# TomasDelaney/A-Deep-Reinforcement-Learning-Enabled-Soft-Exoskeleton-for-Parkinson-s-Patients

Measured on AMD Instinct MI355X. Metric: env steps/sec (batched exo sim) + TD7 grad-steps/sec at 1/2/4/8 MI355X, higher is better.
Workload: dtype f64 sim + bf16 TD7

## Files before the change

a-deep-reinforcement-learning-enabled-soft-exoskeleton-for-parkinson-s-patients_amd/csrc/exo_env.hip:

```cpp
#include <hip/hip_runtime.h>

#include <cmath>
#include <cstdio>
#include <cstring>
#include <string>
#include <vector>

#include "exo_amd.h"
#include "exo_model.h"

using namespace exo;

namespace {

__device__ __forceinline__ double cfg(const Dev &S, int k, int e) { return S.cfg[(size_t)k * S.N + e]; }

__device__ __forceinline__ double wave_min(double v) {
#pragma unroll
    for (int o = 32; o > 0; o >>= 1) v = fmin(v, __shfl_xor(v, o, 64));
    return v;
}
__device__ __forceinline__ double wave_max(double v) {
#pragma unroll
    for (int o = 32; o > 0; o >>= 1) v = fmax(v, __shfl_xor(v, o, 64));
    return v;
}

struct Draws {
    const double *buf;
    uint64_t seed;
    uint32_t env, episode;
    __device__ __forceinline__ double operator()(int p) const {
        return buf ? buf[p] : philox_u01(seed, env, episode, (uint32_t)p);
    }
};

template <int n>
__device__ __forceinline__ void invert(double *a , double *inv) {
#pragma unroll
    for (int i = 0; i < n * n; ++i) inv[i] = (i % (n + 1) == 0) ? 1.0 : 0.0;
#pragma unroll
    for (int k = 0; k < n; ++k) {
        int p = k;
        double best = fabs(a[k * n + k]);
#pragma unroll
        for (int i = k + 1; i < n; ++i) {
            const double v = fabs(a[i * n + k]);
            if (v > best) { best = v; p = i; }
        }
#pragma unroll
        for (int i = k + 1; i < n; ++i) {
            const bool sw = p == i;
#pragma unroll
            for (int j = 0; j < n; ++j) {
                const double t = a[k * n + j], u = inv[k * n + j];
                a[k * n + j] = sw ? a[i * n + j] : t;
                a[i * n + j] = sw ? t : a[i * n + j];
                inv[k * n + j] = sw ? inv[i * n + j] : u;
                inv[i * n + j] = sw ? u : inv[i * n + j];
            }
        }
        const double r = 1.0 / a[k * n + k];
#pragma unroll
        for (int j = 0; j < n; ++j) { a[k * n + j] *= r; inv[k * n + j] *= r; }
#pragma unroll
        for (int i = 0; i < n; ++i) {
            if (i == k) continue;
            const double m = a[i * n + k];
#pragma unroll
            for (int j = 0; j < n; ++j) { a[i * n + j] -= m * a[k * n + j]; inv[i * n + j] -= m * inv[k * n + j]; }
        }
    }
}

template <int EPW, int TS>
__device__ void reset_group(const Dev &S, const Urdf &U, int e, const double *draws, uint64_t seed, float *obs) {
#pragma clang fp contract(off)
    constexpr int NT = EPW * TS, NW = NT / 64;
    static_assert(NT % 64 == 0 && 64 % EPW == 0, "whole wavefronts, a slot's threads spread over lanes");
    const int el = threadIdx.x % EPW, tl = threadIdx.x / EPW, w = threadIdx.x / 64;
    const bool on = e >= 0;
    const int ee = on ? e : 0;
    if (on && tl == 0 && S.pend) S.pend[e] = 0;
    const int N = S.N, L = on ? S.L[ee] : 0, seq = S.seq[ee];
    const uint32_t ep = S.episode[ee];
    const Draws D{draws, seed, (uint32_t)ee, ep};
// ... 97 lines not shown
        const double sr = cfg(S, C_SHIFT, ee);
        for (int j = tl; j < 42; j += TS) {
            const double v = -sr + (sr - (-sr)) * D(pI + 147 + j);
            sShift[el][j] = v;
            S.shift[(size_t)j * N + e] = v;
        }
    }
    __syncthreads();
    if (on) {
        for (int k = tl; k < NSYM; k += TS) {
            int r = 0, c = 0;
#pragma unroll
            for (int q = 0; q < NSYM; ++q)
                if (q == k) { r = SYM_R[q]; c = SYM_C[q]; }
            S.dnz[(size_t)k * N + e] = sD[el][r * 7 + c];
            S.snz[(size_t)k * N + e] = sS[el][r * 7 + c];
        }
        if (tl == 0) {
            double a3[9], i3[9], a4[16], i4[16];
            for (int i = 0; i < 3; ++i)
                for (int j = 0; j < 3; ++j) a3[i * 3 + j] = sI[el][B1[i] * 7 + B1[j]];
            for (int i = 0; i < 4; ++i)
                for (int j = 0; j < 4; ++j) a4[i * 4 + j] = sI[el][B2[i] * 7 + B2[j]];
            invert<3>(a3, i3);
            invert<4>(a4, i4);
            for (int i = 0; i < 3; ++i)
                for (int j = i; j < 3; ++j) sInv[el][B1U[i][j]] = i3[i * 3 + j];
            for (int i = 0; i < 4; ++i)
                for (int j = i; j < 4; ++j) sInv[el][B2U[i][j]] = i4[i * 4 + j];
        }
    }
    __syncthreads();
    if (!on) return;
    for (int k = tl; k < NINV; k += TS) S.iinv[(size_t)k * N + e] = sInv[el][k];
    if (tl != 0) return;
    const double ar = cfg(S, C_ACTR, e), lo = 1 - ar, hi = 1 + ar;
    const double maxS = cfg(S, C_MAXS0, e) * (lo + (hi - lo) * D(pI + 189));
    const double maxE = cfg(S, C_MAXE0, e) * (lo + (hi - lo) * D(pI + 190));
    S.maxSE[e] = maxS;
    S.maxSE[(size_t)N + e] = maxE;
    S.counts[e] = 2;
    S.episode[e] = ep + 1;

    double q[5], act[14][3], ref[6], refc[6];
#pragma unroll
    for (int j = 0; j < 5; ++j) q[j] = S.phys_q[(size_t)j * N + e];
#pragma unroll
    for (int j = 0; j < 6; ++j) refc[j] = S.ref[(size_t)j * N + e];
    link_coms(U, q, act, ref);
    float *o = obs ? obs + (size_t)e * OBS : nullptr;
    float ob[OBS];
#pragma unroll
    for (int i = 0; i < 14; ++i) ob[i] = 0.0f;
    const double tn[4] = {10, 10, 10, 5};
#pragma unroll
    for (int t = 0; t < 3; ++t)
#pragma unroll
        for (int i = 0; i < 4; ++i) ob[14 + t * 4 + i] = (float)(sTrem[el][t][i] / tn[i]);
#pragma unroll
    for (int j = 0; j < 7; ++j)
#pragma unroll
        for (int a = 0; a < 3; ++a) {
            const double p = act[2 * j + 1][a] + sShift[el][(2 * j + 1) * 3 + a];
            const double rc = (j < 2) ? refc[3 + a] : refc[a];
            const double rn = (j < 2) ? ref[3 + a] : ref[a];
            ob[26 + j * 3 + a] = (float)(p - rc);
            const float pv = (float)(p - rn);
            ob[47 + j * 3 + a] = pv;
            S.posv[(size_t)(j * 3 + a) * N + e] = pv;
        }
#pragma unroll
    for (int j = 0; j < 6; ++j) {
        ob[68 + j] = (float)ref[j];
        ob[74 + j] = (float)ref[j];
        S.ref[(size_t)j * N + e] = ref[j];
    }
    if (o) {
#pragma unroll
        for (int i = 0; i < OBS; i += 4) *reinterpret_cast<float4 *>(o + i) = make_float4(ob[i], ob[i + 1], ob[i + 2], ob[i + 3]);
    }
}

constexpr int RESET_EPW = 16, RESET_TS = 32;
__global__ __launch_bounds__(RESET_EPW *RESET_TS) void exo_reset_kernel(Dev S, Urdf U, const uint8_t *mask,
                                                                        const int32_t *ids, int n,
                                                                        const double *draws, int draw_stride,
                                                                        uint64_t seed, float *obs) {
    const int slot = blockIdx.x * RESET_EPW + (int)threadIdx.x % RESET_EPW;
    int e = -1;
    if (ids) {
        if (slot < n) e = ids[slot];
    } else if (slot < S.N && !(mask && !mask[slot])) {
        e = slot;
    }
    reset_group<RESET_EPW, RESET_TS>(S, U, e, draws && slot < n ? draws + (size_t)slot * draw_stride : nullptr,
                                     seed, obs);
}

__global__ __launch_bounds__(64) void exo_reset_list_kernel(Dev S, Urdf U, const int32_t *ids,
                                                            const int32_t *n_ids, uint64_t seed, float *obs) {
    const int n = *n_ids;
    for (int k = blockIdx.x; k < n; k += gridDim.x) reset_group<1, 64>(S, U, ids[k], nullptr, seed, obs);
}

__global__ __launch_bounds__(256) void exo_step_kernel(Dev S, Urdf U, const float *__restrict__ act,
                                                       float *__restrict__ obs, float *__restrict__ rew,
                                                       uint8_t *__restrict__ done, float *__restrict__ info,
                                                       const uint8_t *__restrict__ active) {
    const int gid = blockIdx.x * blockDim.x + threadIdx.x;
    const int e = gid >> 1, role = gid & 1;
    if (e >= S.N) return;
    const int N = S.N, c = S.counts[e], L = S.L[e];
    if ((active && !active[e]) || c >= L - 1) return;

    double T[7];
    {
        const double maxS = S.maxSE[e], maxE = S.maxSE[(size_t)N + e];
        double F[7];
        const float *a = act + (size_t)e * ACT;
#pragma unroll
        for (int j = 0; j < 7; ++j) F[j] = (((double)a[j] + 1) / 2) * (j < 2 ? maxE : maxS);
        double q[5], ak[14][3], refn[6], refo[6];
#pragma unroll
        for (int j = 0; j < 5; ++j) q[j] = S.phys_q[(size_t)j * N + e];
#pragma unroll
        for (int j = 0; j < 6; ++j) refo[j] = S.ref[(size_t)j * N + e];
        if (S.mb_q) {
            double qp[14];
#pragma unroll
            for (int j = 0; j < 14; ++j) qp[j] = S.mb_q[(size_t)(5 + j) * N + e];
            link_coms(U, q, ak, refn, qp);
        } else {
            link_coms(U, q, ak, refn);
        }
#pragma unroll
        for (int k = 0; k < 14; ++k)
#pragma unroll
            for (int a3 = 0; a3 < 3; ++a3) ak[k][a3] += S.shift[(size_t)(k * 3 + a3) * N + e];

        double tau[7][3];
#pragma unroll
        for (int j = 0; j < 7; ++j) {
            const double *k1 = ak[2 * j], *k2 = ak[2 * j + 1];
            const double dx = (k2[0] + 5) - (k1[0] + 5), dy = (k2[1] + 5) - (k1[1] + 5), dz = (k2[2] + 5) - (k1[2] + 5);
            const double fx = cos_atan2(dy, dx) * F[j], fy = cos_atan2(dx, dy) * F[j], fz = cos_atan2(dz, dx) * F[j];
            const double *rn = (j < 2) ? &refn[3] : &refn[0];
            const double r0 = rn[0] - k2[0], r1 = rn[1] - k2[1], r2 = rn[2] - k2[2];
            tau[j][0] = fy * r2 - fz * r1;
            tau[j][1] = fz * r0 - fx * r2;
            tau[j][2] = fx * r1 - fy * r0;
        }
        double at[4];
        at[0] = tau[2][1] + tau[3][1] + tau[4][1] + tau[6][1] + tau[5][1];
        at[1] = tau[2][0] + tau[3][0] + tau[4][0] + tau[6][0] + tau[5][0];
        at[2] = tau[2][2] + tau[3][2] + tau[4][2] + tau[6][2] + tau[5][2];
        at[3] = fabs(tau[0][1]) - fabs(tau[1][1]);

        double tr[7], Ta[7];
#pragma unroll
        for (int j = 0; j < 7; ++j) {
            tr[j] = S.tremor[((size_t)c * 7 + j) * N + e];
            Ta[j] = tr[j] + (j < 4 ? at[j] : 0.0);
            T[j] = role == 0 ? Ta[j] : tr[j];
        }

        if (role == 0) {
// ... 239 lines not shown
__global__ void eval_metrics_kernel(Dev S, const float *__restrict__ info, const uint8_t *__restrict__ stepped,
                                    double L1, double L2, float *__restrict__ counters) {
    const int e = blockIdx.x * blockDim.x + threadIdx.x;
    if (e >= S.N || (stepped && !stepped[e])) return;
    const float *in = info + (size_t)e * INFO;
    const int seq = S.seq[e];
    bool all_sup = true, any_sup = false;
    for (int j = 0; j < 7; ++j) {
        if (!((seq >> j) & 1)) continue;
        const double ref = in[21 + j];
        double tr = (fabs((double)in[7 + j]) - fabs(ref)) / fabs(ref + 1e-10) * 100.0;
        if (!isfinite(tr)) tr = 0.0;
        all_sup &= tr <= 0.0;
        any_sup |= tr <= 0.0;
    }
    const int cnt = S.counts[e];
    const double *imu = S.imu + (size_t)S.motion[e] * 5 * S.Lmax;
    const int col[5] = {2, 3, 4, 0, 1};
    double q0[7], q1[7], q2[7];
    for (int j = 0; j < 7; ++j) {
        const int js = j == 0 ? 1 : (j == 1 ? 0 : j);
        const double o = j < 5 ? imu[col[j] * S.Lmax + cnt] * (PI / 180) : 0.0;
        q0[j] = o;
        q1[j] = (double)in[14 + js] * (PI / 180) + o;
        q2[j] = (double)in[28 + js] * (PI / 180) + o;
    }
    double p0[3], p1[3], p2[3];
    dh_end_effector(q0, L1, L2, p0);
    dh_end_effector(q1, L1, L2, p1);
    dh_end_effector(q2, L1, L2, p2);
    const double ds = sqrt((p1[0] - p0[0]) * (p1[0] - p0[0]) + (p1[1] - p0[1]) * (p1[1] - p0[1]) +
                           (p1[2] - p0[2]) * (p1[2] - p0[2]));
    const double du = sqrt((p2[0] - p0[0]) * (p2[0] - p0[0]) + (p2[1] - p0[1]) * (p2[1] - p0[1]) +
                           (p2[2] - p0[2]) * (p2[2] - p0[2]));
    const double total = (ds - du) / du * 100.0;
    float *cn = counters + (size_t)e * 5;
    if (all_sup) cn[0] += 1;
    if (any_sup) cn[1] += 1;
    if (total < 0) {
        cn[2] += 1;
        cn[4] += (float)total;
    } else {
        cn[3] += 1;
    }
}

__global__ __launch_bounds__(1024) void active_advance_kernel(const uint8_t *__restrict__ table, int rows, int n,
                                                              long long *k, uint8_t *__restrict__ active,
                                                              int32_t *count, const float *__restrict__ rew,
                                                              double *__restrict__ score) {
    __shared__ int wsum[16];
    const long long k0 = *k;
    const long long kk = k0 + 1 < rows ? k0 + 1 : rows - 1;
    int c = 0;
    for (int e = threadIdx.x; e < n; e += blockDim.x) {
        const uint8_t v = table[(size_t)kk * n + e];
        if (score) score[e] += active[e] ? (double)rew[e] : 0.0;
        active[e] = v;
        c += v != 0;
    }
    for (int o = 32; o > 0; o >>= 1) c += __shfl_xor(c, o, 64);
    if ((threadIdx.x & 63) == 0) wsum[threadIdx.x >> 6] = c;
    __syncthreads();
    if (threadIdx.x == 0) {
        *k = kk;
        if (count) {
            int t = 0;
            for (int w = 0; w < (int)(blockDim.x >> 6); ++w) t += wsum[w];
            *count = t;
        }
    }
}

struct exo_ctx {
    int device = 0;
    int N = 0, n_motions = 0, Lmax = 0;
    uint64_t seed = 0;
    Dev S{};
    Urdf U{};
    std::vector<int32_t> L_host, motion_host;
    std::vector<double> imu_host;
    std::vector<void *> allocs;
    float *obs_scratch = nullptr;
    int step_variant = EXO_STEP_AUTO;
    int physics = EXO_PHYS_IDEAL;
    MbModel mb{};
    double *mb_q = nullptr, *mb_qd = nullptr, *mb_tgt = nullptr;
    uint8_t *mb_flag = nullptr;
    unsigned long long *step_clock = nullptr;
    std::string err;
};

namespace {

struct DeviceGuard {
    int prev = -1;
    explicit DeviceGuard(int dev) {
        if (hipGetDevice(&prev) == hipSuccess && prev != dev) (void)hipSetDevice(dev);
        else prev = -1;
    }
    ~DeviceGuard() {
        if (prev >= 0) (void)hipSetDevice(prev);
    }
};

int fail(exo_ctx *c, int code, const std::string &msg) {
    if (c) c->err = msg;
    return code;
}

int check(exo_ctx *c, hipError_t e, const char *what) {
    if (e == hipSuccess) return EXO_OK;
    return fail(c, EXO_EDEVICE, std::string(what) + ": " + hipGetErrorString(e));
}

template <class T>
T *dalloc(exo_ctx *c, size_t n) {
    void *p = nullptr;
    if (hipMalloc(&p, n * sizeof(T)) != hipSuccess) return nullptr;
    (void)hipMemset(p, 0, n * sizeof(T));
    c->allocs.push_back(p);
    return static_cast<T *>(p);
}

}

namespace {
template <class T>
int read1(exo_ctx *c, const T *base, size_t idx, T *out) {
    return check(c, hipMemcpy(out, base + idx, sizeof(T), hipMemcpyDeviceToHost), "read-back");
}
template <class T>
int write1(exo_ctx *c, T *base, size_t idx, T v) {
    return check(c, hipMemcpy(base + idx, &v, sizeof(T), hipMemcpyHostToDevice), "write");
}
}

extern "C" {

int exo_create(const exo_env_config *cfgs, int32_t n_envs, const double *motion_angles, const int32_t *motion_lengths,
               int32_t n_motions, int32_t max_len, uint64_t seed, int32_t device, exo_ctx **out) {
    if (!out || !cfgs || !motion_angles || !motion_lengths || n_envs <= 0 || n_motions <= 0 || max_len <= 2 ||
        max_len > MAX_L)
        return EXO_EINVAL;
    *out = nullptr;
    for (int m = 0; m < n_motions; ++m)
        if (motion_lengths[m] < 4 || motion_lengths[m] > max_len) return EXO_EINVAL;
    std::vector<double> cfg((size_t)C_COUNT * n_envs);
    std::vector<int32_t> seq(n_envs), L(n_envs), mot(n_envs);
    for (int e = 0; e < n_envs; ++e) {
        const exo_env_config &c = cfgs[e];
        if (c.motion < 0 || c.motion >= n_motions) return EXO_EINVAL;
        int bits = 0, n = 0;
        for (int i = 0; i < 7; ++i) {
            if (c.tremor_sequence[i] != 0 && c.tremor_sequence[i] != 1) return EXO_EINVAL;
            bits |= c.tremor_sequence[i] << i;
            n += c.tremor_sequence[i];
        }
        if (n == 0) return EXO_EINVAL;
        seq[e] = bits;
        mot[e] = c.motion;
        L[e] = motion_lengths[c.motion];
        const double v[C_COUNT] = {c.tremor_amplitude_range[0], c.tremor_amplitude_range[1],
                                   c.first_harmonics_interval[0], c.first_harmonics_interval[1],
                                   c.second_harmonics_interval[0], c.second_harmonics_interval[1],
                                   c.max_force_shoulder, c.max_force_elbow, c.dr_actuator_end_pos_shift,
                                   c.dr_actuator_range, c.matrix_noise_fraction,
                                   n * 0.5 + 0.9 + 0.05 + 0.05 + 0.5, (double)n};
        for (int k = 0; k < C_COUNT; ++k) cfg[(size_t)k * n_envs + e] = v[k];
    }
    exo_ctx *c = new exo_ctx();
    c->device = device;
    c->N = n_envs;
    c->n_motions = n_motions;
    c->Lmax = max_len;
    c->seed = seed;
    c->L_host = L;
    c->motion_host = mot;
    c->imu_host.assign(motion_angles, motion_angles + (size_t)n_motions * 5 * max_len);
    build_urdf(c->U);
    DeviceGuard g(device);
    const size_t N = n_envs;
    Dev &S = c->S;
    S.N = n_envs; S.n_motions = n_motions; S.Lmax = max_len;
    int32_t *motion_d = dalloc<int32_t>(c, N), *L_d = dalloc<int32_t>(c, N), *seq_d = dalloc<int32_t>(c, N);
    double *cfg_d = dalloc<double>(c, cfg.size()), *imu_d = dalloc<double>(c, c->imu_host.size());
    S.tremor = dalloc<double>(c, (size_t)max_len * 7 * N);
    S.iinv = dalloc<double>(c, NINV * N);
    S.dnz = dalloc<double>(c, NSYM * N);
    S.snz = dalloc<double>(c, NSYM * N);
    S.shift = dalloc<double>(c, 42 * N);
    S.maxSE = dalloc<double>(c, 2 * N);
    S.episode = dalloc<uint32_t>(c, N);
    S.counts = dalloc<int32_t>(c, N);
    S.phys_q = dalloc<double>(c, 5 * N);
    S.ref = dalloc<double>(c, 6 * N);
    S.posv = dalloc<float>(c, 21 * N);
    S.prev_a = dalloc<double>(c, 7 * N);
    S.prev2_a = dalloc<double>(c, 7 * N);
    S.err = dalloc<int32_t>(c, 1);
    S.viol = dalloc<int32_t>(c, N);
    c->obs_scratch = dalloc<float>(c, N * OBS);
    for (void *p : c->allocs)
        if (!p) { exo_destroy(c); return EXO_ENOMEM; }
    if (!motion_d || !L_d || !seq_d || !cfg_d || !imu_d || !S.tremor || !S.iinv ||
        !S.dnz || !S.snz || !S.shift || !S.maxSE || !S.episode || !S.counts || !S.phys_q || !S.ref || !S.posv ||
        !S.prev_a || !S.prev2_a || !S.err || !S.viol || !c->obs_scratch) {
        exo_destroy(c);
        return EXO_ENOMEM;
    }
    S.motion = motion_d; S.L = L_d; S.seq = seq_d; S.cfg = cfg_d; S.imu = imu_d;
    exo_set_tremor_model(c, nullptr, EXO_TREMOR_SIGN_PER_SAMPLE);
    hipError_t e = hipMemcpy(motion_d, mot.data(), N * 4, hipMemcpyHostToDevice);
    if (e == hipSuccess) e = hipMemcpy(L_d, L.data(), N * 4, hipMemcpyHostToDevice);
    if (e == hipSuccess) e = hipMemcpy(seq_d, seq.data(), N * 4, hipMemcpyHostToDevice);
    if (e == hipSuccess) e = hipMemcpy(cfg_d, cfg.data(), cfg.size() * 8, hipMemcpyHostToDevice);
    if (e == hipSuccess) e = hipMemcpy(imu_d, c->imu_host.data(), c->imu_host.size() * 8, hipMemcpyHostToDevice);
    if (e != hipSuccess) { exo_destroy(c); return EXO_EDEVICE; }
    int rc = exo_reset(c, nullptr, c->obs_scratch, nullptr);
    if (rc == EXO_OK) rc = check(c, hipDeviceSynchronize(), "exo_create");
    if (rc != EXO_OK) { exo_destroy(c); return rc; }
    *out = c;
    return EXO_OK;
}

int exo_reset(exo_ctx *c, const uint8_t *mask_dev, float *obs_dev, void *stream) {
    if (!c) return EXO_EINVAL;
    DeviceGuard g(c->device);
    hipLaunchKernelGGL(exo_reset_kernel, dim3((c->N + RESET_EPW - 1) / RESET_EPW), dim3(RESET_EPW * RESET_TS), 0,
                       (hipStream_t)stream, c->S, c->U, mask_dev, (const int32_t *)nullptr, 0,
                       (const double *)nullptr, 0, c->seed, obs_dev);
    return check(c, hipGetLastError(), "exo_reset");
}

int exo_reset_from_draws(exo_ctx *c, const int32_t *env_ids_host, int32_t n, const double *draws_host, float *obs_dev,
                         void *stream) {
    if (!c || !env_ids_host || !draws_host || n <= 0) return EXO_EINVAL;
    for (int k = 0; k < n; ++k)
        if (env_ids_host[k] < 0 || env_ids_host[k] >= c->N) return fail(c, EXO_EINVAL, "env id out of range");
    DeviceGuard g(c->device);
    const int stride = EXO_DRAWS_PER_EPISODE(c->Lmax);
    int32_t *ids = nullptr;
    double *dr = nullptr;
    if (hipMalloc(&ids, n * 4) != hipSuccess || hipMalloc(&dr, (size_t)n * stride * 8) != hipSuccess) {
        (void)hipFree(ids);
        return fail(c, EXO_ENOMEM, "exo_reset_from_draws: out of memory");
    }
    hipStream_t s = (hipStream_t)stream;
    hipError_t e = hipMemcpyAsync(ids, env_ids_host, n * 4, hipMemcpyHostToDevice, s);
    if (e == hipSuccess) e = hipMemcpyAsync(dr, draws_host, (size_t)n * stride * 8, hipMemcpyHostToDevice, s);
    if (e == hipSuccess) {
        hipLaunchKernelGGL(exo_reset_kernel, dim3((n + RESET_EPW - 1) / RESET_EPW), dim3(RESET_EPW * RESET_TS), 0,
                           s, c->S, c->U, (const uint8_t *)nullptr, ids, n, dr, stride, c->seed, obs_dev);
        e = hipGetLastError();
    }
    if (e == hipSuccess) e = hipStreamSynchronize(s);
    (void)hipFree(ids);
    (void)hipFree(dr);
    return check(c, e, "exo_reset_from_draws");
}

namespace {
__global__ void step_clock_kernel(unsigned long long *clk, int end) {
    const unsigned long long t = wall_clock64();
    if (!end) {
        clk[0] = t;
    } else {
        clk[1] += t - clk[0];
        clk[2] += 1;
    }
}
}

int exo_step(exo_ctx *c, const float *act_dev, float *obs_dev, float *rew_dev, uint8_t *done_dev, float *info_dev,
             const uint8_t *active_dev, void *stream) {
    return exo_step_carry(c, act_dev, obs_dev, rew_dev, done_dev, info_dev, active_dev, nullptr, stream);
}

namespace {
bool rows_variant(const exo_ctx *c) {
    return c->step_variant == EXO_STEP_ROWS_SHARED || c->step_variant == EXO_STEP_ROWS ||
           (c->step_variant == EXO_STEP_AUTO && c->N <= 16384);
}

__global__ __launch_bounds__(1024) void budget_advance_kernel(const int32_t *counts, const int32_t *L,
                                                              const uint8_t *pend, int n, uint8_t *active,
                                                              int32_t *count, int32_t *remaining,
                                                              long long *steps_total) {
    __shared__ int wsum[2][16];
    int a = 0, rem = 0;
    for (int e = threadIdx.x; e < n; e += blockDim.x) {
        const bool run = counts[e] < L[e] - 1, p = pend[e] != 0;
        active[e] = run && !p;
        a += run && !p;
        rem += run || p;
    }
    for (int o = 32; o > 0; o >>= 1) {
        a += __shfl_xor(a, o, 64);
        rem += __shfl_xor(rem, o, 64);
    }
    if ((threadIdx.x & 63) == 0) {
        wsum[0][threadIdx.x >> 6] = a;
        wsum[1][threadIdx.x >> 6] = rem;
    }
    __syncthreads();
    if (threadIdx.x == 0) {
        int ta = 0, tr = 0;
        for (int w = 0; w < (int)(blockDim.x >> 6); ++w) {
            ta += wsum[0][w];
            tr += wsum[1][w];
        }
        if (steps_total) *steps_total += *count;
        *count = ta;
        *remaining = tr;
    }
}

__global__ __launch_bounds__(1024) void episode_advance_kernel(const int32_t *counts, const int32_t *L,
                                                               const uint8_t *pend, int n, uint8_t *active,
                                                               int32_t *count, int32_t *reset_ids,
                                                               long long *steps_total) {
    __shared__ int wsum[16];
    __shared__ int nres;
    if (threadIdx.x == 0) nres = 0;
    __syncthreads();
    int a = 0;
    for (int e = threadIdx.x; e < n; e += blockDim.x) {
        const bool fin = counts[e] >= L[e] - 1, p = pend && pend[e] != 0;
        if (fin && !p) reset_ids[atomicAdd(&nres, 1)] = e;
        const bool run = !p;
        active[e] = run;
        a += run;
    }
    for (int o = 32; o > 0; o >>= 1) a += __shfl_xor(a, o, 64);
    if ((threadIdx.x & 63) == 0) wsum[threadIdx.x >> 6] = a;
    __syncthreads();
    if (threadIdx.x == 0) {
        int ta = 0;
        for (int w = 0; w < (int)(blockDim.x >> 6); ++w) ta += wsum[w];
        if (steps_total) *steps_total += *count;
        *count = ta;
        reset_ids[n] = nres;
    }
}
}

int exo_set_step_budget(exo_ctx *c, int32_t budget) {
    if (!c || budget < 0) return EXO_EINVAL;
    DeviceGuard g(c->device);
    if (budget > 0 && (!rows_variant(c) || c->physics != EXO_PHYS_IDEAL))
        return fail(c, EXO_EINVAL, "exo_set_step_budget: row-parallel step kernels and idealised physics only");
    int rc = check(c, hipDeviceSynchronize(), "exo_set_step_budget");
    if (rc) return rc;
    if (budget == 0) {
        if (c->S.pend) {
            std::vector<uint8_t> p(c->N);
            rc = check(c, hipMemcpy(p.data(), c->S.pend, c->N, hipMemcpyDeviceToHost), "exo_set_step_budget");
            if (rc) return rc;
            for (uint8_t v : p)
                if (v) return fail(c, EXO_EINVAL, "exo_set_step_budget: a solve is still pending");
        }
        c->S.budget = 0;
        return EXO_OK;
    }
    if (!c->S.pend) {
        c->S.pend = dalloc<uint8_t>(c, c->N);
        c->S.rk = dalloc<double>(c, (size_t)RK_FIELDS * c->N);
        if (!c->S.pend || !c->S.rk) return fail(c, EXO_ENOMEM, "exo_set_step_budget: out of memory");
    }
    c->S.budget = budget;
    return EXO_OK;
}

int exo_budget_advance(exo_ctx *c, uint8_t *active_dev, int32_t *count_dev, int32_t *remaining_dev,
                       int64_t *steps_total_dev, void *stream) {
    if (!c || !active_dev || !count_dev || !remaining_dev) return EXO_EINVAL;
    if (!c->S.pend) return fail(c, EXO_EINVAL, "exo_budget_advance: no step budget set");
    DeviceGuard g(c->device);
    hipLaunchKernelGGL(budget_advance_kernel, dim3(1), dim3(1024), 0, (hipStream_t)stream, c->S.counts, c->S.L,
                       c->S.pend, c->N, active_dev, count_dev, remaining_dev, (long long *)steps_total_dev);
    return check(c, hipGetLastError(), "exo_budget_advance");
}

int exo_episode_advance(exo_ctx *c, uint8_t *active_dev, int32_t *count_dev, int32_t *reset_ws_dev,
                        int64_t *steps_total_dev, float *obs_dev, void *stream) {
    if (!c || !active_dev || !count_dev || !reset_ws_dev || !obs_dev) return EXO_EINVAL;
    DeviceGuard g(c->device);
    const hipStream_t s = (hipStream_t)stream;
    hipLaunchKernelGGL(episode_advance_kernel, dim3(1), dim3(1024), 0, s, c->S.counts, c->S.L, c->S.pend, c->N,
                       active_dev, count_dev, reset_ws_dev, (long long *)steps_total_dev);
    hipError_t e = hipGetLastError();
    if (e == hipSuccess) {
        hipLaunchKernelGGL(exo_reset_list_kernel, dim3(std::min(c->N, 64)), dim3(64), 0, s, c->S, c->U, reset_ws_dev,
                           reset_ws_dev + c->N, c->seed, obs_dev);
        e = hipGetLastError();
    }
    return check(c, e, "exo_episode_advance");
}

int exo_step_carry(exo_ctx *c, const float *act_dev, float *obs_dev, float *rew_dev, uint8_t *done_dev,
                   float *info_dev, const uint8_t *active_dev, const float *obs_cur_dev, void *stream) {
    if (!c || !act_dev || !obs_dev || !rew_dev || !done_dev) return EXO_EINVAL;
    DeviceGuard g(c->device);
    const bool shared = c->step_variant == EXO_STEP_ROWS_SHARED;
    const bool rows = rows_variant(c);
    if (c->S.budget > 0 && (!rows || c->physics != EXO_PHYS_IDEAL))
        return fail(c, EXO_EINVAL, "exo_step: the step budget needs the row-parallel kernel and idealised physics");
    hipError_t e = hipSuccess;
    if (c->step_clock) {
        hipLaunchKernelGGL(step_clock_kernel, dim3(1), dim3(1), 0, (hipStream_t)stream, c->step_clock, 0);
        e = hipGetLastError();
    }
    if (e != hipSuccess) {
    } else if (rows) {
        e = launch_exo_step_rp(c->S, c->U, act_dev, obs_dev, rew_dev, done_dev, info_dev, active_dev,
                               (hipStream_t)stream, shared, obs_cur_dev);
    } else {
        const int threads = 256, lanes = 2 * c->N;
        hipLaunchKernelGGL(exo_step_kernel, dim3((lanes + threads - 1) / threads), dim3(threads), 0,
                           (hipStream_t)stream, c->S, c->U, act_dev, obs_dev, rew_dev, done_dev, info_dev, active_dev);
        e = hipGetLastError();
    }
    if (e == hipSuccess && c->physics == EXO_PHYS_MULTIBODY)
        e = launch_exo_multibody(c->S, c->U, c->mb, c->S.mb_tgt, c->S.mb_flag, 1, (hipStream_t)stream);
    if (e == hipSuccess && c->step_clock) {
        hipLaunchKernelGGL(step_clock_kernel, dim3(1), dim3(1), 0, (hipStream_t)stream, c->step_clock, 1);
        e = hipGetLastError();
    }
    return check(c, e, "exo_step");
}

void exo_multibody_default_params(exo_mb_params *p) {
    if (!p) return;
    p->gravity = 9.81;
    p->kp = 0.1;
    p->kd = 1.0;
    p->motor_impulse = 1e5 * DT;
    p->passive_impulse = 1.0;
    p->limit_impulse = 100.0;
    p->erp = 0.2;
    p->lin_damp = 0.04;
    p->ang_damp = 0.04;
    p->max_vel = 100.0;
    p->iters = 50;
}

int exo_set_physics(exo_ctx *c, int32_t mode, const exo_mb_params *params) {
    if (!c || (mode != EXO_PHYS_IDEAL && mode != EXO_PHYS_MULTIBODY)) return EXO_EINVAL;
    if (mode == EXO_PHYS_MULTIBODY && c->S.budget > 0)
        return fail(c, EXO_EINVAL, "exo_set_physics: the step budget needs idealised physics");
    exo_mb_params p;
    exo_multibody_default_params(&p);
    if (params) p = *params;
    if (p.iters < 0 || p.iters > 100000 || !(p.motor_impulse >= 0) || !(p.passive_impulse >= 0) ||
        !(p.limit_impulse >= 0) || !(p.max_vel > 0))
        return fail(c, EXO_EINVAL, "exo_set_physics: invalid multibody parameters");
    DeviceGuard g(c->device);
    const size_t N = c->N;
    int rc = check(c, hipDeviceSynchronize(), "exo_set_physics");
    if (rc) return rc;
    if (mode == EXO_PHYS_IDEAL) {
        c->physics = mode;
        c->S.mb_q = c->S.mb_qd = c->S.mb_tgt = nullptr;
        c->S.mb_flag = nullptr;
        return EXO_OK;
    }
    if (!c->mb_q) {
        c->mb_q = dalloc<double>(c, NJ * N);
        c->mb_qd = dalloc<double>(c, NJ * N);
        c->mb_tgt = dalloc<double>(c, 5 * N);
        c->mb_flag = dalloc<uint8_t>(c, N);
// ... 265 lines not shown
```

a-deep-reinforcement-learning-enabled-soft-exoskeleton-for-parkinson-s-patients_amd/csrc/lap.hip:

```cpp
#include <hip/hip_runtime.h>

#include <algorithm>
#include <cstdint>
#include <cstdlib>
#include <string>

#include "lap_chain.h"
#include "philox.h"
#include "exo_amd.h"

namespace {

constexpr int UPD_THREADS = 1024;

__device__ __forceinline__ float *stratum_tree(float *tree, int s, int cap) { return tree + (size_t)s * 2 * cap; }

constexpr int TOPN = 8192;
template <int NTOP = TOPN>
__device__ bool propagate_top(float *T, int cap, int levels, const int32_t *slot, int n, float *top) {
    int lv = 1;
    for (; lv <= levels && ((2 * cap) >> lv) > NTOP / 2; ++lv) {
        __syncthreads();
        for (int k = threadIdx.x; k < n; k += blockDim.x) {
            const int node = (cap + slot[k]) >> lv;
            T[node] = T[2 * node] + T[2 * node + 1];
        }
    }
    __syncthreads();
    if (lv > levels) return false;
    const int lim = min(NTOP, 2 * cap);
    if (blockDim.x == UPD_THREADS) {
        constexpr int PER = NTOP / UPD_THREADS;
        float v[PER];
#pragma unroll
        for (int j = 0; j < PER; ++j) {
            const int i = threadIdx.x + j * UPD_THREADS;
            v[j] = i < lim ? T[i] : 0.0f;
        }
#pragma unroll
        for (int j = 0; j < PER; ++j) {
            const int i = threadIdx.x + j * UPD_THREADS;
            if (i < lim) top[i] = v[j];
        }
    } else {
        for (int i = threadIdx.x; i < lim; i += blockDim.x) top[i] = T[i];
    }
    for (; lv <= levels; ++lv) {
        __syncthreads();
        for (int k = threadIdx.x; k < n; k += blockDim.x) {
            const int node = (cap + slot[k]) >> lv;
            top[node] = top[2 * node] + top[2 * node + 1];
        }
    }
    __syncthreads();
    const int wb = min(NTOP / 2, cap);
    for (int i = 1 + threadIdx.x; i < wb; i += blockDim.x) T[i] = top[i];
    __syncthreads();
    return true;
}
__device__ void propagate(float *T, int cap, int levels, const int32_t *slot, int n) {
    __shared__ float top[TOPN];
    propagate_top(T, cap, levels, slot, n, top);
}

__device__ void propagate_span(float *T, int cap, int levels, int capacity, int first, int count) {
    __shared__ float top[TOPN];
    if (count <= 0) return;
    int a0 = first, e0 = first + count, a1 = 0, e1 = 0;
    if (count >= capacity) {
        a0 = 0;
        e0 = capacity;
    } else if (e0 > capacity) {
        e1 = e0 - capacity;
        e0 = capacity;
    }
    int lv = 1;
    for (; lv <= levels && ((2 * cap) >> lv) > TOPN / 2; ++lv) {
        __syncthreads();
        const int lo0 = (cap + a0) >> lv, n0 = ((cap + e0 - 1) >> lv) - lo0 + 1;
        const int lo1 = (cap + a1) >> lv, n1 = e1 > a1 ? ((cap + e1 - 1) >> lv) - lo1 + 1 : 0;
        for (int k = threadIdx.x; k < n0 + n1; k += blockDim.x) {
            const int node = k < n0 ? lo0 + k : lo1 + k - n0;
            T[node] = T[2 * node] + T[2 * node + 1];
        }
    }
    __syncthreads();
    if (lv > levels) return;
    const int lim = min(TOPN, 2 * cap);
    for (int i = threadIdx.x; i < lim; i += blockDim.x) top[i] = T[i];
    for (; lv <= levels; ++lv) {
        __syncthreads();
        const int lo0 = (cap + a0) >> lv, n0 = ((cap + e0 - 1) >> lv) - lo0 + 1;
        const int lo1 = (cap + a1) >> lv, n1 = e1 > a1 ? ((cap + e1 - 1) >> lv) - lo1 + 1 : 0;
        for (int k = threadIdx.x; k < n0 + n1; k += blockDim.x) {
            const int node = k < n0 ? lo0 + k : lo1 + k - n0;
            top[node] = top[2 * node] + top[2 * node + 1];
        }
    }
    __syncthreads();
    const int wb = min(TOPN / 2, cap);
    for (int i = 1 + threadIdx.x; i < wb; i += blockDim.x) T[i] = top[i];
    __syncthreads();
}

constexpr int SPAN_LDS = 4096;
constexpr int SPAN_LEVELS = 32;
__device__ bool propagate_span_lds(float *T, int cap, int levels, int capacity, int first, int count,
                                   float *buf , float *edge ) {
    const int a = cap + first, e = cap + first + count - 1;
    if (count <= 0 || first + count > capacity || count > SPAN_LDS - 2 || levels >= SPAN_LEVELS) return false;
    const int t = threadIdx.x;
    if (t < 2 * levels) {
        const int lv = t >> 1, right = t & 1;
        const int lo = a >> lv, hi = e >> lv;
        if (!right && (lo & 1)) edge[t] = T[lo - 1];
        if (right && !(hi & 1)) edge[t] = T[hi + 1];
    }
    float *A = buf, *B = buf + SPAN_LDS;
    {
        const int base = a & ~1;
        for (int c = a + t; c <= e; c += blockDim.x) A[c - base] = T[c];
    }
    __syncthreads();
    if (t == 0) {
        if (a & 1) A[0] = edge[0];
        if (!(e & 1)) A[(e | 1) - (a & ~1)] = edge[1];
    }
    for (int lv = 1; lv <= levels; ++lv) {
        __syncthreads();
        const int lo = a >> lv, hi = e >> lv, cbase = (a >> (lv - 1)) & ~1, nbase = lo & ~1;
        for (int node = lo + t; node <= hi; node += blockDim.x) {
            const int c = 2 * node - cbase;
            const float v = A[c] + A[c + 1];
            T[node] = v;
            B[node - nbase] = v;
        }
        if (t == 0 && lv < levels) {
            if (lo & 1) B[0] = edge[2 * lv];
            if (!(hi & 1)) B[(hi | 1) - nbase] = edge[2 * lv + 1];
        }
        float *tmp = A;
        A = B;
        B = tmp;
    }
    __syncthreads();
    return true;
}

constexpr int ADD_CHUNK = 4096;
__global__ __launch_bounds__(UPD_THREADS) void lap_add_kernel(float *tree, const float *maxp, int cap, int levels,
                                                              int capacity, const int32_t *stratum,
                                                              const int32_t *slot, int n) {
    const int s = blockIdx.x;
    float *T = stratum_tree(tree, s, cap);
    __shared__ int32_t mine[ADD_CHUNK];
    __shared__ int count;
    const float p = *maxp;
    for (int base = 0; base < n; base += ADD_CHUNK) {
        if (threadIdx.x == 0) count = 0;
        __syncthreads();
        const int end = min(n, base + ADD_CHUNK);
        for (int k = base + threadIdx.x; k < end; k += blockDim.x) {
            if (stratum[k] != s) continue;
            const int sl = slot[k];
            if (sl < 0 || sl >= capacity) continue;
            T[cap + sl] = p;
            mine[atomicAdd(&count, 1)] = sl;
        }
        __syncthreads();
        propagate(T, cap, levels, mine, count);
    }
}

constexpr int MAXLV = 24;
template <class At>
__device__ __forceinline__ float prefix_sum(At at, int cap, int levels, int sz) {
    if (sz >= cap) return at(1);
    float v[MAXLV];
#pragma unroll
    for (int j = 0; j < MAXLV; ++j) {
        v[j] = 0.0f;
        if (j < levels) {
            const int lv = levels - 1 - j;
            const float x = at(2 * ((1 << j) | (sz >> (lv + 1))));
            v[j] = ((sz >> lv) & 1) ? x : 0.0f;
// ... 597 lines not shown
            const int r = rk[jj];
            if (jj + 1 == m) {
                carry_r = r;
                carry_i = ri[jj];
                carry_J = soff + jj;
                sl[jj] = -1;
                continue;
            }
            const long long mr = mult_below(count0 + r, E);
            const bool win = (long long)rk[jj + 1] > mr * E - count0;
            const int slot = win ? slot_of(r) : -1;
            sl[jj] = slot;
            if (win && part == 0) T[cap + slot] = p;
        }
        __syncthreads();
        if (cpart >= 0) {
            const int j0 = ((cpart - soff) % KC + KC) % KC;
            copy_rows<VEC>(st, state, action, next_state, reward, done, action_scale, ri, sl, s, capacity, j0, KC, m,
                           t, UPD_THREADS);
        }
        offset += chunk_tot;
        soff += m;
        __syncthreads();
    }
    if (t == 0) {
        carry_slot = -1;
        if (carry_r >= 0) {
            carry_slot = slot_of(carry_r);
            if (part == 0) T[cap + carry_slot] = p;
        }
    }
    __syncthreads();
    if (carry_slot >= 0 && wv == 0 && carry_J % KC == cpart)
        copy_rows<VEC>(st, state, action, next_state, reward, done, action_scale, &carry_i, &carry_slot, s, capacity,
                       0, 1, 1, lane, 64);
    const int n_act = offset;
    if (part == 0 && n_act > 0) {
        __shared__ float span_buf[2 * SPAN_LDS], span_edge[2 * SPAN_LEVELS];
        __syncthreads();
        const long long last = mult_below(count0 + n_act - 1, E) - m0;
        const int cnt = (int)min(last + 1, (long long)capacity);
        if (!propagate_span_lds(T, cap, levels, capacity, (int)ptr0, cnt, span_buf, span_edge))
            propagate_span(T, cap, levels, capacity, (int)ptr0, cnt);
    }
    __syncthreads();
    __shared__ int last;
    if (t == 0) {
        last = atomicAdd(ticket, 1u) == (uint32_t)(E * K - 1);
        if (last) {
            const long long na = mult_below(count0 + n_act, E) - m0;
            const long long size = min(size0 + na, (long long)capacity);
            for (int q = 0; q < E; ++q) ring_size[q] = (int32_t)size;
            ref[0] = (ptr0 + na) % capacity;
            ref[1] = count0 + n_act;
            ref[2] = size;
            *ticket = 0u;
        }
    }
    __syncthreads();
    if (!last || !adv.table) return;
    const long long k0 = *adv.k;
    const long long kk = k0 + 1 < adv.rows ? k0 + 1 : adv.rows - 1;
    int c = 0;
    for (int e = t; e < n; e += UPD_THREADS) {
        const uint8_t v = adv.table[(size_t)kk * n + e];
        if (adv.score) adv.score[e] += adv.active[e] ? (double)reward[e] : 0.0;
        adv.active[e] = v;
        c += v != 0;
    }
    for (int o = 32; o > 0; o >>= 1) c += __shfl_xor(c, o, 64);
    __shared__ int wc[UPD_THREADS / 64];
    if (lane == 0) wc[wv] = c;
    __syncthreads();
    if (t == 0) {
        *adv.k = kk;
        if (adv.count) {
            int tot = 0;
            for (int w = 0; w < UPD_THREADS / 64; ++w) tot += wc[w];
            *adv.count = tot;
        }
    }
}

__global__ __launch_bounds__(256) void lap_store_copy_kernel(lap_storage_desc st, const float *state,
                                                             const float *action, const float *next_state,
                                                             const float *reward, const uint8_t *done,
                                                             float action_scale, int n, const int32_t *row_of) {
    const int i = blockIdx.x * 4 + (threadIdx.x >> 6), lane = threadIdx.x & 63;
    if (i >= n) return;
    const long r = row_of[i];
    if (r < 0) return;
    const int sd = st.state_dim, ad = st.action_dim;
    for (int k = lane; k < sd; k += 64) {
        st.state[r * sd + k] = state[(long)i * sd + k];
        st.next_state[r * sd + k] = next_state[(long)i * sd + k];
    }
    for (int k = lane; k < ad; k += 64) st.action[r * ad + k] = action[(long)i * ad + k] / action_scale;
    if (lane == 0) {
        st.reward[r] = reward[i];
        st.not_done[r] = 1.0f - (done[i] ? 1.0f : 0.0f);
    }
}

__device__ __forceinline__ void sample_descend(const float *tree, int cap, int levels, int capacity, float ud,
                                               const int32_t *size, int batch, int d, int lane, int32_t *idx,
                                               const lap_storage_desc &st, float *o_state, float *o_action,
                                               float *o_next, float *o_reward, float *o_not_done) {
    const int s = d / batch;
    const float *T = tree + (size_t)s * 2 * cap;
    const int sz = size[s];
    const float val = ud * prefix_total(T, cap, levels, sz);
    const int node = descend_from([T](int n) { return T[n]; }, val, 1, 0, levels);
    int i = node - cap;
    if (i >= sz) i = sz > 0 ? sz - 1 : 0;
    if (lane == 0) idx[d] = i;
    const long r = (long)s * (capacity + 1) + i;
    const int sd = st.state_dim, ad = st.action_dim;
    for (int k = lane; k < sd; k += 64) {
        o_state[(long)d * sd + k] = st.state[r * sd + k];
        o_next[(long)d * sd + k] = st.next_state[r * sd + k];
    }
    for (int k = lane; k < ad; k += 64) o_action[(long)d * ad + k] = st.action[r * ad + k];
    if (lane == 0) {
        o_reward[d] = st.reward[r];
        o_not_done[d] = st.not_done[r];
    }
}

struct SampleRng {
    uint64_t seed;
    uint32_t tag;
    unsigned long long *counter;
    uint32_t *ticket;
};

__global__ __launch_bounds__(256) void lap_sample_gather_kernel(const float *tree, int cap, int levels, int capacity,
                                                                const float *u, const int32_t *size, int batch,
                                                                int total, int32_t *idx, lap_storage_desc st,
                                                                float *o_state, float *o_action, float *o_next,
                                                                float *o_reward, float *o_not_done, SampleRng rng) {
    const int d = blockIdx.x * 4 + (threadIdx.x >> 6), lane = threadIdx.x & 63;
    if (rng.counter) {
        const unsigned long long call = *rng.counter;
        __syncthreads();
        if (threadIdx.x == 0) {
            __threadfence();
            if (atomicAdd(rng.ticket, 1u) == gridDim.x - 1) {
                *rng.counter = call + 1ull;
                *rng.ticket = 0u;
            }
        }
        if (d >= total) return;
        uint32_t r[4];
        philox_block(rng.seed, rng.tag, call, (uint32_t)d, r);
        sample_descend(tree, cap, levels, capacity, u01_open_hi(r[0]), size, batch, d, lane, idx, st, o_state,
                       o_action, o_next, o_reward, o_not_done);
        return;
    }
    if (d >= total) return;
    sample_descend(tree, cap, levels, capacity, u[d], size, batch, d, lane, idx, st, o_state, o_action, o_next,
                   o_reward, o_not_done);
}


#ifndef LAP_TOPN_US
#define LAP_TOPN_US 8192
// ... 589 lines not shown

extern "C" {

int32_t lap_tree_floats(int32_t n_strata, int32_t capacity) {
    int cap = 1;
    while (cap < capacity) cap <<= 1;
    return n_strata * 2 * cap;
}

int lap_init(const lap_tree_desc *t, void *stream) {
    if (!valid(t)) return EXO_EINVAL;
    hipError_t e = hipMemsetAsync(t->tree, 0, (size_t)t->n_strata * 2 * t->cap * sizeof(float), (hipStream_t)stream);
    if (e != hipSuccess) return EXO_EDEVICE;
    hipLaunchKernelGGL(lap_init_kernel, dim3(1), dim3(1), 0, (hipStream_t)stream, t->max_priority);
    return rc(hipGetLastError());
}

int lap_add(const lap_tree_desc *t, const int32_t *stratum, const int32_t *slot, int32_t n, void *stream) {
    if (!valid(t) || !stratum || !slot || n < 0) return EXO_EINVAL;
    if (n == 0) return EXO_OK;
    hipLaunchKernelGGL(lap_add_kernel, dim3(t->n_strata), dim3(UPD_THREADS), 0, (hipStream_t)stream, t->tree,
                       t->max_priority, t->cap, levels_of(t), t->capacity, stratum, slot, n);
    return rc(hipGetLastError());
}

int lap_sample(const lap_tree_desc *t, const float *u, const int32_t *size, int32_t batch, int32_t *idx, void *stream) {
    if (!valid(t) || !u || !size || !idx || batch <= 0) return EXO_EINVAL;
    const int th = 128;
    hipLaunchKernelGGL(lap_sample_kernel, dim3((batch + th - 1) / th, t->n_strata), dim3(th), 0, (hipStream_t)stream,
                       t->tree, t->cap, levels_of(t), u, size, batch, idx);
    return rc(hipGetLastError());
}

int lap_update(const lap_tree_desc *t, const int32_t *idx, const float *prio, int32_t batch, void *stream) {
    if (!valid(t) || !idx || !prio || batch <= 0) return EXO_EINVAL;
    hipLaunchKernelGGL(lap_update_kernel, dim3(t->n_strata), dim3(UPD_THREADS), 0, (hipStream_t)stream, t->tree,
                       t->max_priority, t->cap, levels_of(t), idx, prio, batch);
    return rc(hipGetLastError());
}

int lap_reset_max(const lap_tree_desc *t, void *stream) {
    if (!valid(t)) return EXO_EINVAL;
    hipError_t e = hipMemsetAsync(t->max_priority, 0, sizeof(float), (hipStream_t)stream);
    if (e != hipSuccess) return EXO_EDEVICE;
    hipLaunchKernelGGL(lap_reset_max_kernel, dim3(256), dim3(1024), 0, (hipStream_t)stream, t->tree, t->max_priority,
                       t->cap, t->n_strata);
    return rc(hipGetLastError());
}

int lap_totals(const lap_tree_desc *t, float *out, void *stream) {
    if (!valid(t) || !out) return EXO_EINVAL;
    hipLaunchKernelGGL(lap_totals_kernel, dim3((t->n_strata + 63) / 64), dim3(64), 0, (hipStream_t)stream, t->tree,
                       t->cap, t->n_strata, out);
    return rc(hipGetLastError());
}

int lap_store_batch(const lap_tree_desc *t, const lap_storage_desc *st, const float *state, const float *action,
                    const float *next_state, const float *reward, const uint8_t *done, const int32_t *strata,
                    const uint8_t *active, float action_scale, int32_t n, int32_t *row_ws, void *stream) {
    if (!valid(t) || !st || !st->state || !st->action || !st->next_state || !st->reward || !st->not_done ||
        !st->ptr || !st->size || st->state_dim <= 0 || st->action_dim <= 0 || !state || !action || !next_state ||
        !reward || !done || !strata || !row_ws || n < 0 || action_scale == 0.0f)
        return EXO_EINVAL;
    if (n == 0) return EXO_OK;
    const char *fused_var = getenv("EXO_LAP_STORE_FUSED");
    const bool fused_env = fused_var && fused_var[0] == '1';
    if (fused_env && n <= STORE_FUSED_MAX && n <= t->capacity) {
        const bool vec = (st->state_dim & 3) == 0 &&
                         ((reinterpret_cast<uintptr_t>(state) | reinterpret_cast<uintptr_t>(next_state) |
                           reinterpret_cast<uintptr_t>(st->state) | reinterpret_cast<uintptr_t>(st->next_state)) &
                          15) == 0;
        if (vec)
            hipLaunchKernelGGL(lap_store_fused_kernel<true>, dim3(t->n_strata), dim3(UPD_THREADS), 0,
                               (hipStream_t)stream, t->tree, t->max_priority, t->cap, levels_of(t), t->capacity,
                               st->ptr, st->size, strata, active, n, row_ws, *st, state, action, next_state, reward,
                               done, action_scale);
        else
            hipLaunchKernelGGL(lap_store_fused_kernel<false>, dim3(t->n_strata), dim3(UPD_THREADS), 0,
                               (hipStream_t)stream, t->tree, t->max_priority, t->cap, levels_of(t), t->capacity,
                               st->ptr, st->size, strata, active, n, row_ws, *st, state, action, next_state, reward,
                               done, action_scale);
        return rc(hipGetLastError());
    }
    if (n > 4 * STORE_CHUNK)
        hipLaunchKernelGGL(lap_store_rank_kernel<16>, dim3(t->n_strata), dim3(UPD_THREADS), 0, (hipStream_t)stream,
                           t->tree, t->max_priority, t->cap, levels_of(t), t->capacity, st->ptr, st->size, strata,
                           active, n, row_ws);
    else
        hipLaunchKernelGGL(lap_store_rank_kernel<4>, dim3(t->n_strata), dim3(UPD_THREADS), 0, (hipStream_t)stream,
                           t->tree, t->max_priority, t->cap, levels_of(t), t->capacity, st->ptr, st->size, strata,
                           active, n, row_ws);
    if (hipGetLastError() != hipSuccess) return EXO_EDEVICE;
    hipLaunchKernelGGL(lap_store_copy_kernel, dim3((n + 3) / 4), dim3(256), 0, (hipStream_t)stream, *st, state,
                       action, next_state, reward, done, action_scale, n, row_ws);
    return rc(hipGetLastError());
}

int lap_store_batch_ref(const lap_tree_desc *t, const lap_storage_desc *st, int64_t *ref_dev, const float *state,
                        const float *action, const float *next_state, const float *reward, const uint8_t *done,
                        const int32_t *strata, const uint8_t *active, float action_scale, int32_t n,
                        int32_t *ws_dev, void *stream) {
    if (!valid(t) || !st || !st->state || !st->action || !st->next_state || !st->reward || !st->not_done ||
        !st->size || st->state_dim <= 0 || st->action_dim <= 0 || !ref_dev || !state || !action || !next_state ||
        !reward || !done || !strata || !ws_dev || n < 0 || action_scale == 0.0f)
        return EXO_EINVAL;
    if (n == 0) return EXO_OK;
    int32_t *rank_row = ws_dev, *slot_of = ws_dev + n, *row_of = ws_dev + 2 * n;
    hipLaunchKernelGGL(lap_store_ref_slots_kernel, dim3(1), dim3(UPD_THREADS), 0, (hipStream_t)stream, t->capacity,
                       t->n_strata, (long long *)ref_dev, st->size, strata, active, n, rank_row, slot_of, row_of);
    if (hipGetLastError() != hipSuccess) return EXO_EDEVICE;
    hipLaunchKernelGGL(lap_add_kernel, dim3(t->n_strata), dim3(UPD_THREADS), 0, (hipStream_t)stream, t->tree,
                       t->max_priority, t->cap, levels_of(t), t->capacity, strata, slot_of, n);
    if (hipGetLastError() != hipSuccess) return EXO_EDEVICE;
    hipLaunchKernelGGL(lap_store_copy_kernel, dim3((n + 3) / 4), dim3(256), 0, (hipStream_t)stream, *st, state,
                       action, next_state, reward, done, action_scale, n, row_of);
    return rc(hipGetLastError());
}

static int store_ref_fused(const lap_tree_desc *t, const lap_storage_desc *st, int64_t *ref_dev,
                           const float *state, const float *action, const float *next_state, const float *reward,
                           const uint8_t *done, const int32_t *strata, const uint8_t *active, float action_scale,
                           int32_t n, uint32_t *ticket_dev, const MaskAdvance &adv, void *stream) {
    if (!valid(t) || !st || !st->state || !st->action || !st->next_state || !st->reward || !st->not_done ||
        !st->size || st->state_dim <= 0 || st->action_dim <= 0 || !ref_dev || !state || !action || !next_state ||
        !reward || !done || !strata || !ticket_dev || n < 0 || action_scale == 0.0f)
        return EXO_EINVAL;
    if (n == 0) return EXO_OK;
    const int E = t->n_strata;
    const int K = 1 + std::max(1, std::min(15, (n + E * 64 - 1) / (E * 64)));
    auto al16 = [](const void *p) { return ((uintptr_t)p & 15u) == 0; };
    const bool vec = st->state_dim % 4 == 0 && al16(state) && al16(next_state) && al16(st->state) &&
                     al16(st->next_state);
    if (vec)
        hipLaunchKernelGGL(lap_store_ref_fused_kernel<true>, dim3(E, K), dim3(UPD_THREADS), 0, (hipStream_t)stream,
                           t->tree, t->max_priority, t->cap, levels_of(t), t->capacity, E, (long long *)ref_dev,
                           st->size, *st, state, action, next_state, reward, done, action_scale, strata, active, n,
                           ticket_dev, adv);
    else
        hipLaunchKernelGGL(lap_store_ref_fused_kernel<false>, dim3(E, K), dim3(UPD_THREADS), 0, (hipStream_t)stream,
                           t->tree, t->max_priority, t->cap, levels_of(t), t->capacity, E, (long long *)ref_dev,
                           st->size, *st, state, action, next_state, reward, done, action_scale, strata, active, n,
                           ticket_dev, adv);
    return rc(hipGetLastError());
}

int lap_store_batch_ref_fused(const lap_tree_desc *t, const lap_storage_desc *st, int64_t *ref_dev,
                              const float *state, const float *action, const float *next_state, const float *reward,
                              const uint8_t *done, const int32_t *strata, const uint8_t *active, float action_scale,
                              int32_t n, uint32_t *ticket_dev, void *stream) {
    return store_ref_fused(t, st, ref_dev, state, action, next_state, reward, done, strata, active, action_scale, n,
                           ticket_dev, MaskAdvance{}, stream);
}

int lap_store_batch_ref_fused_adv(const lap_tree_desc *t, const lap_storage_desc *st, int64_t *ref_dev,
                                  const float *state, const float *action, const float *next_state,
                                  const float *reward, const uint8_t *done, const int32_t *strata, uint8_t *active,
                                  float action_scale, int32_t n, uint32_t *ticket_dev, const uint8_t *table,
                                  int32_t rows, int64_t *k_dev, int32_t *count_dev, double *score_dev, void *stream) {
    if (!table || rows <= 0 || !k_dev || !active) return EXO_EINVAL;
    return store_ref_fused(t, st, ref_dev, state, action, next_state, reward, done, strata, active, action_scale, n,
                           ticket_dev, MaskAdvance{table, rows, (long long *)k_dev, active, count_dev, score_dev},
                           stream);
}

int lap_sample_gather(const lap_tree_desc *t, const lap_storage_desc *st, const float *u, int32_t batch,
                      int32_t *idx, float *out_state, float *out_action, float *out_next_state, float *out_reward,
// ... 127 lines not shown
```

Measured before the change: 18.17 million.

## Fuse episode advance with resets and LAP store rank+copy into single kernels

Episode advance now runs as one grid-wide kernel. Each 64-lane block computes its active flags, resets finished environments in place, and the last-arriving block sums the active count through a ticket counter. This replaces a single-block scan followed by a separate reset launch. LAP buffer storage for small batches likewise fuses rank assignment, tree leaf writes, span propagation and row copying into one 2D-grid kernel, with extra blocks splitting the copy work. Both paths are on by default behind env vars; they cut launches and serialization but depend on atomic tickets and on reusing the tree's slot 0 as a counter.

```diff
diff --git a/a-deep-reinforcement-learning-enabled-soft-exoskeleton-for-parkinson-s-patients_amd/csrc/exo_env.hip b/a-deep-reinforcement-learning-enabled-soft-exoskeleton-for-parkinson-s-patients_amd/csrc/exo_env.hip
--- a/a-deep-reinforcement-learning-enabled-soft-exoskeleton-for-parkinson-s-patients_amd/csrc/exo_env.hip
+++ b/a-deep-reinforcement-learning-enabled-soft-exoskeleton-for-parkinson-s-patients_amd/csrc/exo_env.hip
@@ -2,6 +2,7 @@
 
 #include <cmath>
 #include <cstdio>
+#include <cstdlib>
 #include <cstring>
 #include <string>
 #include <vector>
@@ -265,6 +266,7 @@
 }
 
 constexpr int RESET_EPW = 16, RESET_TS = 32;
+constexpr int ADV_EPW = 64;
 __global__ __launch_bounds__(RESET_EPW *RESET_TS) void exo_reset_kernel(Dev S, Urdf U, const uint8_t *mask,
                                                                         const int32_t *ids, int n,
                                                                         const double *draws, int draw_stride,
@@ -670,6 +672,7 @@
     std::vector<double> imu_host;
     std::vector<void *> allocs;
     float *obs_scratch = nullptr;
+    int32_t *adv_ws = nullptr;
     int step_variant = EXO_STEP_AUTO;
     int physics = EXO_PHYS_IDEAL;
     MbModel mb{};
@@ -789,6 +792,7 @@
     S.err = dalloc<int32_t>(c, 1);
     S.viol = dalloc<int32_t>(c, N);
     c->obs_scratch = dalloc<float>(c, N * OBS);
+    c->adv_ws = dalloc<int32_t>(c, (N + ADV_EPW - 1) / ADV_EPW + 1);
     for (void *p : c->allocs)
         if (!p) { exo_destroy(c); return EXO_ENOMEM; }
     if (!motion_d || !L_d || !seq_d || !cfg_d || !imu_d || !S.tremor || !S.iinv ||
@@ -931,6 +935,41 @@
         reset_ids[n] = nres;
     }
 }
+
+__global__ __launch_bounds__(ADV_EPW) void episode_advance_one_kernel(Dev S, Urdf U, int n, uint8_t *active,
+                                                                      int32_t *count, int32_t *ws,
+                                                                      long long *steps_total, uint64_t seed,
+                                                                      float *obs) {
+    const int lane = threadIdx.x, e0 = blockIdx.x * ADV_EPW, e = e0 + lane, G = gridDim.x;
+    bool run = false, fin = false;
+    if (e < n) {
+        const bool p = S.pend && S.pend[e] != 0;
+        fin = S.counts[e] >= S.L[e] - 1 && !p;
+        run = !p;
+        active[e] = run;
+    }
+    const int a = __popcll(__ballot(run));
+    for (unsigned long long fm = __ballot(fin); fm; fm &= fm - 1)
+        reset_group<1, ADV_EPW>(S, U, e0 + __ffsll((long long)fm) - 1, nullptr, seed, obs);
+    __shared__ int last;
+    uint32_t *ticket = reinterpret_cast<uint32_t *>(ws + G);
+    if (lane == 0) {
+        ws[blockIdx.x] = a;
+        __threadfence();
+        last = atomicAdd(ticket, 1u) == (uint32_t)(G - 1);
+    }
+    __syncthreads();
+    if (!last) return;
+    __threadfence();
+    int tot = 0;
+    for (int b = lane; b < G; b += ADV_EPW) tot += __builtin_nontemporal_load(ws + b);
+    for (int o = 32; o > 0; o >>= 1) tot += __shfl_xor(tot, o, 64);
+    if (lane == 0) {
+        if (steps_total) *steps_total += *count;
+        *count = tot;
+        *ticket = 0u;
+    }
+}
 }
 
 int exo_set_step_budget(exo_ctx *c, int32_t budget) {
@@ -975,6 +1014,13 @@
     if (!c || !active_dev || !count_dev || !reset_ws_dev || !obs_dev) return EXO_EINVAL;
     DeviceGuard g(c->device);
     const hipStream_t s = (hipStream_t)stream;
+    const char *one_var = getenv("EXO_EPISODE_ADVANCE_ONE");
+    if (!(one_var && one_var[0] == '0')) {
+        hipLaunchKernelGGL(episode_advance_one_kernel, dim3((c->N + ADV_EPW - 1) / ADV_EPW), dim3(ADV_EPW), 0, s,
+                           c->S, c->U, c->N, active_dev, count_dev, c->adv_ws, (long long *)steps_total_dev, c->seed,
+                           obs_dev);
+        return check(c, hipGetLastError(), "exo_episode_advance");
+    }
     hipLaunchKernelGGL(episode_advance_kernel, dim3(1), dim3(1024), 0, s, c->S.counts, c->S.L, c->S.pend, c->N,
                        active_dev, count_dev, reset_ws_dev, (long long *)steps_total_dev);
     hipError_t e = hipGetLastError();
diff --git a/a-deep-reinforcement-learning-enabled-soft-exoskeleton-for-parkinson-s-patients_amd/csrc/lap.hip b/a-deep-reinforcement-learning-enabled-soft-exoskeleton-for-parkinson-s-patients_amd/csrc/lap.hip
--- a/a-deep-reinforcement-learning-enabled-soft-exoskeleton-for-parkinson-s-patients_amd/csrc/lap.hip
+++ b/a-deep-reinforcement-learning-enabled-soft-exoskeleton-for-parkinson-s-patients_amd/csrc/lap.hip
@@ -63,8 +63,7 @@
     propagate_top(T, cap, levels, slot, n, top);
 }
 
-__device__ void propagate_span(float *T, int cap, int levels, int capacity, int first, int count) {
-    __shared__ float top[TOPN];
+__device__ void propagate_span_in(float *T, int cap, int levels, int capacity, int first, int count, float *top) {
     if (count <= 0) return;
     int a0 = first, e0 = first + count, a1 = 0, e1 = 0;
     if (count >= capacity) {
@@ -101,6 +100,10 @@
     const int wb = min(TOPN / 2, cap);
     for (int i = 1 + threadIdx.x; i < wb; i += blockDim.x) T[i] = top[i];
     __syncthreads();
+}
+__device__ void propagate_span(float *T, int cap, int levels, int capacity, int first, int count) {
+    __shared__ float top[TOPN];
+    propagate_span_in(T, cap, levels, capacity, first, count, top);
 }
 
 constexpr int SPAN_LDS = 4096;
@@ -864,6 +867,103 @@
     }
 }
 
+constexpr int STORE_ONE_MAX = 2 * STORE_CHUNK;
+constexpr int STORE_ONE_ROWS = 64;
+
+template <bool VEC>
+__global__ __launch_bounds__(UPD_THREADS) void lap_store_one_kernel(
+    float *tree, const float *maxp, int cap, int levels, int capacity, int32_t *ring_ptr, int32_t *ring_size,
+    const int32_t *strata, const uint8_t *active, int n, int32_t *row_of, lap_storage_desc st, const float *state,
+    const float *action, const float *next_state, const float *reward, const uint8_t *done, float action_scale) {
+    const int s = blockIdx.x, part = blockIdx.y, K = gridDim.y;
+    const int t = threadIdx.x, lane = t & 63, wv = t >> 6;
+    __shared__ int wsum[UPD_THREADS / 64];
+    __shared__ int chunk_total;
+    static_assert(2 * STORE_CHUNK == 2 * SPAN_LDS && 2 * SPAN_LDS == TOPN, "one buffer: ri | sl, span levels, top");
+    __shared__ float lds[2 * SPAN_LDS];
+    __shared__ float span_edge[2 * SPAN_LEVELS];
+    int32_t *ri = reinterpret_cast<int32_t *>(lds), *sl = ri + STORE_CHUNK;
+    float *T = stratum_tree(tree, s, cap);
+    const int KC = K > 1 ? K - 1 : 1, cpart = K > 1 ? part - 1 : 0;
+    const float p = *maxp;
+    const int ptr0 = ring_ptr[s], size0 = ring_size[s];
+    const int row0 = s * (capacity + 1);
+    int offset = 0;
+    for (int base = 0; base < n; base += STORE_CHUNK) {
+        int stk[4], cnt = 0;
+        bool f[4];
+#pragma unroll
+        for (int k = 0; k < 4; ++k) {
+            const int i = base + 4 * t + k;
+            stk[k] = i < n ? strata[i] : -1;
+            f[k] = i < n && (!active || active[i]);
+        }
+#pragma unroll
+        for (int k = 0; k < 4; ++k) {
+            f[k] = f[k] && stk[k] == s;
+            cnt += f[k];
+        }
+        int incl = cnt;
+#pragma unroll
+        for (int o = 1; o < 64; o <<= 1) {
+            const int v = __shfl_up(incl, o, 64);
+            if (lane >= o) incl += v;
+        }
+        if (lane == 63) wsum[wv] = incl;
+        __syncthreads();
+        if (t == 0) {
+            int acc = 0;
+            for (int k = 0; k < UPD_THREADS / 64; ++k) {
+                const int v = wsum[k];
+                wsum[k] = acc;
+                acc += v;
+            }
+            chunk_total = acc;
+        }
+        __syncthreads();
+        int j = wsum[wv] + incl - cnt;
+#pragma unroll
+        for (int k = 0; k < 4; ++k) {
+            const int i = base + 4 * t + k;
+            if (i >= n) continue;
+            if (part == 0) {
+                if (s == 0 && (stk[k] < 0 || stk[k] >= (int)gridDim.x)) row_of[i] = -1;
+                if (stk[k] == s && !f[k]) row_of[i] = row0 + capacity;
+            }
+            if (f[k]) {
+                const int slot = (ptr0 + offset + j) % capacity;
+                ri[j] = i;
+                sl[j] = slot;
+                if (part == 0) T[cap + slot] = p;
+                ++j;
+            }
+        }
+        __syncthreads();
+        const int m = chunk_total;
+        if (cpart >= 0) {
+            const int j0 = ((cpart - offset) % KC + KC) % KC;
+            for (int jj = j0 + t * KC; jj < m; jj += UPD_THREADS * KC) row_of[ri[jj]] = row0 + sl[jj];
+            copy_rows<VEC>(st, state, action, next_state, reward, done, action_scale, ri, sl, s, capacity, j0, KC, m, t,
+                           UPD_THREADS);
+        }
+        offset += m;
+        __syncthreads();
+    }
+    if (part == 0) {
+        if (!propagate_span_lds(T, cap, levels, capacity, ptr0, offset, lds, span_edge))
+            propagate_span_in(T, cap, levels, capacity, ptr0, offset, lds);
+    }
+    if (t == 0) {
+        uint32_t *ticket = reinterpret_cast<uint32_t *>(T);
+        __threadfence();
+        if (atomicAdd(ticket, 1u) == (uint32_t)(K - 1)) {
+            ring_ptr[s] = (ptr0 + offset) % capacity;
+            ring_size[s] = min(size0 + offset, capacity);
+            *ticket = 0u;
+        }
+    }
+}
+
 __global__ __launch_bounds__(256) void lap_store_copy_kernel(lap_storage_desc st, const float *state,
                                                              const float *action, const float *next_state,
                                                              const float *reward, const uint8_t *done,
@@ -1619,6 +1719,24 @@
                                done, action_scale);
         return rc(hipGetLastError());
     }
+    const char *one_var = getenv("EXO_LAP_STORE_ONE");
+    if (!(one_var && one_var[0] == '0') && n <= STORE_ONE_MAX && n <= t->capacity) {
+        const int E = t->n_strata;
+        int K = 1 + std::max(1, std::min(15, (n + E * STORE_ONE_ROWS - 1) / (E * STORE_ONE_ROWS)));
+        if (const char *kv = getenv("EXO_LAP_STORE_ONE_K")) K = std::max(1, std::min(16, atoi(kv)));
+        auto al16 = [](const void *p) { return ((uintptr_t)p & 15u) == 0; };
+        const bool vec = st->state_dim % 4 == 0 && al16(state) && al16(next_state) && al16(st->state) &&
+                         al16(st->next_state);
+        if (vec)
+            hipLaunchKernelGGL(lap_store_one_kernel<true>, dim3(E, K), dim3(UPD_THREADS), 0, (hipStream_t)stream,
+                               t->tree, t->max_priority, t->cap, levels_of(t), t->capacity, st->ptr, st->size, strata,
+                               active, n, row_ws, *st, state, action, next_state, reward, done, action_scale);
+        else
+            hipLaunchKernelGGL(lap_store_one_kernel<false>, dim3(E, K), dim3(UPD_THREADS), 0, (hipStream_t)stream,
+                               t->tree, t->max_priority, t->cap, levels_of(t), t->capacity, st->ptr, st->size, strata,
+                               active, n, row_ws, *st, state, action, next_state, reward, done, action_scale);
+        return rc(hipGetLastError());
+    }
     if (n > 4 * STORE_CHUNK)
         hipLaunchKernelGGL(lap_store_rank_kernel<16>, dim3(t->n_strata), dim3(UPD_THREADS), 0, (hipStream_t)stream,
                            t->tree, t->max_priority, t->cap, levels_of(t), t->capacity, st->ptr, st->size, strata,
```

Result: no change. 18.13 million, median of 3 (-0.2%).
